# yongxuUSTC/DNN-for-speech-enhancement

Measured on AMD Instinct MI355X. Metric: training frames/sec (257x11 input, 3x2048 DNN), higher is better.
Workload: dtype f32; 1 GPU; C2: 2827->2048->2048->2048->257 ReLU+dropout(0.1/0.2), fp32, 256 frames/GPU/step (global bunch 256), lrate 1, momentum 0.5, 102400-frame chunk resident in HBM; parallelism=dp1, global_bunch=256, exchange=none, launcher=single process

## Files before the change

### dnn-for-speech-enhancement_amd/csrc/bp_device.h

```cpp
#pragma once
#include <hip/hip_runtime.h>
#include <stdint.h>

#include <type_traits>
#include <utility>

typedef float f32x16 __attribute__((ext_vector_type(16)));

template <int B, int E, class F>
__device__ __forceinline__ void static_for(F &&f)
{
    if constexpr (B < E) {
        f(std::integral_constant<int, B>{});
        static_for<B + 1, E>(std::forward<F>(f));
    }
}

__device__ __forceinline__ void philox4x32_10(uint32_t &c0, uint32_t &c1, uint32_t &c2, uint32_t &c3,
                                              uint32_t k0, uint32_t k1)
{
#pragma unroll
    for (int r = 0; r < 10; ++r) {
        const uint32_t h0 = __umulhi(0xD2511F53u, c0), l0 = 0xD2511F53u * c0;
        const uint32_t h1 = __umulhi(0xCD9E8D57u, c2), l1 = 0xCD9E8D57u * c2;
        const uint32_t n0 = h1 ^ c1 ^ k0, n2 = h0 ^ c3 ^ k1;
        c0 = n0; c1 = l1; c2 = n2; c3 = l0;
        k0 += 0x9E3779B9u; k1 += 0xBB67AE85u;
    }
}

__device__ __forceinline__ void drop_words4(uint32_t (&w)[4], int r0, int n, int frame_off, uint32_t n_true, uint32_t layer,
                                            uint32_t step, uint32_t seed_lo, uint32_t seed_hi)
{
    const uint64_t g0 = (uint64_t)(uint32_t)(r0 + frame_off);
    const uint64_t idx = (g0 >> 2) * (uint64_t)n_true + (uint32_t)n;
    uint32_t a[4] = {(uint32_t)idx, (uint32_t)(idx >> 32), layer, step};
    philox4x32_10(a[0], a[1], a[2], a[3], seed_lo, seed_hi);
    const int sh = frame_off & 3;
    if (sh == 0) { w[0] = a[0]; w[1] = a[1]; w[2] = a[2]; w[3] = a[3]; return; }
    const uint64_t idx2 = idx + (uint64_t)n_true;
    uint32_t b[4] = {(uint32_t)idx2, (uint32_t)(idx2 >> 32), layer, step};
    philox4x32_10(b[0], b[1], b[2], b[3], seed_lo, seed_hi);
    if (sh == 1) { w[0] = a[1]; w[1] = a[2]; w[2] = a[3]; w[3] = b[0]; }
    else if (sh == 2) { w[0] = a[2]; w[1] = a[3]; w[2] = b[0]; w[3] = b[1]; }
    else { w[0] = a[3]; w[1] = b[0]; w[2] = b[1]; w[3] = b[2]; }
}

__device__ __forceinline__ float act_fwd(int act, float x)
{
    return act == 0 ? (x > 0.0f ? x : 0.0f) : 1.0f / (1.0f + expf(-x));
}
__device__ __forceinline__ float act_bwd(int act, float y)
{
    return act == 0 ? (y > 0.0f ? 1.0f : 0.0f) : (1.0f - y) * y;
}

__device__ __forceinline__ float update_delta(float mom, float c1, float wc, float ndiv, float d, float g, float w)
{
    return mom * d - c1 * (g / ndiv + wc * w);
}

__device__ __forceinline__ bool last_arrival(unsigned *ticket, unsigned *lds_word, unsigned n)
{
    asm volatile("s_waitcnt vmcnt(0)" ::: "memory");
    __syncthreads();
    if (threadIdx.x == 0) *lds_word = __hip_atomic_fetch_add(ticket, 1u, __ATOMIC_RELAXED, __HIP_MEMORY_SCOPE_AGENT);
    __syncthreads();
    return (*lds_word & (n - 1)) == n - 1;
}
```

### dnn-for-speech-enhancement_amd/csrc/bp_kernels.h

```cpp
#pragma once
#include <hip/hip_runtime.h>
#include <stddef.h>
#include <stdint.h>

#include "bp_device.h"

enum { EPI_FWD_HIDDEN = 0, EPI_FWD_OUT = 1, EPI_DGRAD = 2, EPI_WGRAD_UPDATE = 3, EPI_WGRAD_STORE = 4,
       EPI_OUT_SPLIT = 6 ,
       EPI_FWD_OUT_LOGI = 7, EPI_OUT_SPLIT_LOGI = 8 };
static constexpr bool epi_out(int epi) { return epi == EPI_FWD_OUT || epi == EPI_FWD_OUT_LOGI; }
static constexpr bool epi_out_split(int epi) { return epi == EPI_OUT_SPLIT || epi == EPI_OUT_SPLIT_LOGI; }
static constexpr int OUT_SPLITS = 4;

struct GemmArgs {
    const float *A, *B;
    int lda, ldb;
    int K;
    int tiles_m, tiles_n;
#ifdef BP_TRACE
    unsigned long long *trace;
#endif
    int k_split;
    size_t slab_stride;
    float *ks_slab; unsigned *ks_ticket;
};

struct EpiArgs {
    float *C; int ldc;
    int m_limit, n_limit;
    int n_true;
    const float *bias;
    float alpha;
    int act;
    const float *aux; int ldaux;
    int lin_cols;
    float *aux2; int ldaux2;
    float scale;
    float mom, c1, wc, ndiv;
    float *bias_w, *bias_d, *bias_g;
    uint32_t drop_thresh, seed_lo, seed_hi, step, layer;
    int frame_off;
    const uint8_t *mask; int ldmask;
    int loss;
    unsigned *done;
};
static_assert(sizeof(EpiArgs) == 160 && offsetof(EpiArgs, aux2) == 56 && offsetof(EpiArgs, done) == 152, "lin_cols / loss must sit in padding");

struct EpiPre { float bias; f32x16 p0, p1; };

template <class T>
__device__ __forceinline__ T *uniform_ptr(T *p)
{
    const unsigned long long v = (unsigned long long)p;
    const unsigned lo = __builtin_amdgcn_readfirstlane((unsigned)v), hi = __builtin_amdgcn_readfirstlane((unsigned)(v >> 32));
    typedef __attribute__((address_space(1))) T *GlobalPtr;
    return (T *)(GlobalPtr)(((unsigned long long)hi << 32) | lo);
}

template <class T>
__device__ __forceinline__ T *sgpr_row_base(T *p)
{
    typedef __attribute__((address_space(1))) T *GlobalPtr;
    GlobalPtr q = (GlobalPtr)p;
    asm volatile("" : "+s"(q));
    return (T *)q;
}

template <int EPI, int R0, int RN>
__device__ __forceinline__ void epilogue_fetch(const EpiArgs &e, int mb, int nb, int lane, EpiPre &p)
{
    if constexpr (EPI == EPI_WGRAD_UPDATE) {
        const int mbc = mb < e.m_limit ? mb : 0;
        const float *cw = uniform_ptr(e.C + (size_t)mbc * e.ldc + nb);
        const float *cd = uniform_ptr(e.aux2 + (size_t)mbc * e.ldc + nb);
        const unsigned ldc = __builtin_amdgcn_readfirstlane(e.ldc);
        const unsigned lob = 4u * ((unsigned)(4 * (lane >> 5)) * (unsigned)e.ldc + (unsigned)(lane & 31));
#pragma unroll
        for (int r = R0; r < R0 + RN; ++r) {
            const unsigned ro = (unsigned)((r & 3) + 8 * (r >> 2)) * ldc;
            p.p0[r] = *reinterpret_cast<const float *>(reinterpret_cast<const char *>(sgpr_row_base(cw + ro)) + lob);
            p.p1[r] = *reinterpret_cast<const float *>(reinterpret_cast<const char *>(sgpr_row_base(cd + ro)) + lob);
        }
        return;
    }
    const int n = nb + (lane & 31);
    const int rbase = mb + 4 * (lane >> 5);
    static_assert(!epi_out_split(EPI), "fetched as EPI_FWD_OUT[_LOGI]");
    if constexpr (EPI == EPI_FWD_HIDDEN || epi_out(EPI)) p.bias = e.bias[n];
    if constexpr (epi_out(EPI) || EPI == EPI_DGRAD) {
        if (epi_out(EPI) && !e.C) return;
#pragma unroll
        for (int r = R0; r < R0 + RN; ++r) {
            const int m = rbase + (r & 3) + 8 * (r >> 2);
            const int mc = m < e.m_limit ? m : e.m_limit - 1;
            p.p0[r] = e.aux[(size_t)mc * e.ldaux + n];
        }
    }
}

template <int EPI, int R0, int RN>
__device__ __forceinline__ void epilogue_block(const EpiArgs &e, int mb, int nb, const f32x16 &acc, int lane,
                                               const EpiPre &p)
{
    static_assert(RN % 4 == 0 && R0 % 4 == 0, "register range must cover whole 4-row groups");
    if constexpr (EPI == EPI_WGRAD_UPDATE || EPI == EPI_WGRAD_STORE) {
        const int n = nb + (lane & 31);
        if (n >= e.n_limit || mb >= e.m_limit) return;
        float *cw = uniform_ptr(e.C + (size_t)mb * e.ldc + nb);
        const unsigned ldc = __builtin_amdgcn_readfirstlane(e.ldc);
        const unsigned lob = 4u * ((unsigned)(4 * (lane >> 5)) * (unsigned)e.ldc + (unsigned)(lane & 31));
#pragma unroll
        for (int r = R0; r < R0 + RN; ++r) {
            const unsigned ro = (unsigned)((r & 3) + 8 * (r >> 2)) * ldc;
            if constexpr (EPI == EPI_WGRAD_UPDATE) {
                float *cd = uniform_ptr(e.aux2 + (size_t)mb * e.ldc + nb);
                const float w = p.p0[r];
                const float d = update_delta(e.mom, e.c1, e.wc, e.ndiv, p.p1[r], acc[r], w);
                *reinterpret_cast<float *>(reinterpret_cast<char *>(sgpr_row_base(cd + ro)) + lob) = d;
                *reinterpret_cast<float *>(reinterpret_cast<char *>(sgpr_row_base(cw + ro)) + lob) = d + 1.0f * w;
            } else {
                __hip_atomic_store(reinterpret_cast<float *>(reinterpret_cast<char *>(sgpr_row_base(cw + ro)) + lob), acc[r], __ATOMIC_RELAXED, __HIP_MEMORY_SCOPE_SYSTEM);
            }
        }
        return;
    }
    const int n = nb + (lane & 31);
    const int rbase = mb + 4 * (lane >> 5);
    if (n >= e.n_limit) return;
    if constexpr (EPI == EPI_FWD_HIDDEN) {
        const float bn = p.bias;
        const bool live = n < e.n_true;
#pragma unroll
        for (int q = R0 / 4; q < (R0 + RN) / 4; ++q) {
            uint32_t w[4] = {0xFFFFFFFFu, 0xFFFFFFFFu, 0xFFFFFFFFu, 0xFFFFFFFFu};
            const int r0 = rbase + 8 * q;
            if (e.mask) {
#pragma unroll
                for (int j = 0; j < 4; ++j) w[j] = (r0 + j < e.m_limit && live && e.mask[(size_t)(r0 + j) * e.ldmask + n]) ? 0u : 0xFFFFFFFFu;
            } else if (e.drop_thresh) drop_words4(w, r0, n, e.frame_off, (uint32_t)e.n_true, e.layer, e.step, e.seed_lo, e.seed_hi);
#pragma unroll
            for (int j = 0; j < 4; ++j) {
                const int m = r0 + j;
                float y = act_fwd(e.act, e.alpha * acc[q * 4 + j] + bn);
                if (!live || w[j] < e.drop_thresh) y = 0.0f;
                if (m < e.m_limit) e.C[(size_t)m * e.ldc + n] = y;
            }
        }
    } else if constexpr (EPI == EPI_FWD_OUT) {
        const float bn = p.bias;
        const bool live = n < e.n_true;
#pragma unroll
        for (int r = R0; r < R0 + RN; ++r) {
            const int m = rbase + (r & 3) + 8 * (r >> 2);
            if (m < e.m_limit) {
                const float o = live ? e.alpha * acc[r] + bn : 0.0f;
                if (e.aux2) e.aux2[(size_t)m * e.ldaux2 + n] = o;
                if (e.C) e.C[(size_t)m * e.ldc + n] = live ? e.scale * (o - p.p0[r]) : 0.0f;
            }
        }
    } else if constexpr (EPI == EPI_FWD_OUT_LOGI) {
        const float bn = p.bias;
        const bool live = n < e.n_true, logi = live && n >= e.lin_cols, chain = logi && e.loss == 1;
#pragma unroll
        for (int r = R0; r < R0 + RN; ++r) {
            const int m = rbase + (r & 3) + 8 * (r >> 2);
            if (m < e.m_limit) {
                const float z = live ? e.alpha * acc[r] + bn : 0.0f;
                const float o = logi ? 1.0f / (1.0f + expf(-z)) : z;
                if (e.aux2) e.aux2[(size_t)m * e.ldaux2 + n] = o;
                if (e.C) {
                    float d = live ? e.scale * (o - p.p0[r]) : 0.0f;
                    if (chain) d *= o * (1.0f - o);
                    e.C[(size_t)m * e.ldc + n] = d;
                }
            }
        }
    } else if constexpr (EPI == EPI_DGRAD) {
#pragma unroll
        for (int r = R0; r < R0 + RN; ++r) {
            const int m = rbase + (r & 3) + 8 * (r >> 2);
            if (m < e.m_limit) e.C[(size_t)m * e.ldc + n] = act_bwd(e.act, p.p0[r]) * acc[r];
        }
    } else {
        static_assert(EPI == EPI_WGRAD_UPDATE || EPI == EPI_WGRAD_STORE, "epilogue without a branch");
    }
}

template <int R0>
__device__ __forceinline__ void out_split_store(const EpiArgs &e, float *slab, int mb, int nb, const f32x16 &acc, int lane)
{
    const int n = nb + (lane & 31), rbase = mb + 4 * (lane >> 5);
    if (n >= e.n_limit) return;
#pragma unroll
    for (int r = R0; r < R0 + 4; ++r) {
        const int m = rbase + (r & 3) + 8 * (r >> 2);
        if (m < e.m_limit) __hip_atomic_store(slab + (size_t)m * e.ldc + n, acc[r], __ATOMIC_RELAXED, __HIP_MEMORY_SCOPE_AGENT);
    }
}
template <int R0>
__device__ __forceinline__ void out_split_sum(const EpiArgs &e, const float *slab0, size_t stride, int mb, int nb, f32x16 &acc, int lane)
{
    const int n = nb + (lane & 31), rbase = mb + 4 * (lane >> 5);
    if (n >= e.n_limit) return;
    float p[OUT_SPLITS][4];
#pragma unroll
    for (int z = 0; z < OUT_SPLITS; ++z)
#pragma unroll
        for (int rr = 0; rr < 4; ++rr) {
            const int r = R0 + rr, m = rbase + (r & 3) + 8 * (r >> 2), mc = m < e.m_limit ? m : e.m_limit - 1;
            p[z][rr] = __hip_atomic_load(slab0 + z * stride + (size_t)mc * e.ldc + n, __ATOMIC_RELAXED, __HIP_MEMORY_SCOPE_AGENT);
        }
#pragma unroll
    for (int rr = 0; rr < 4; ++rr) {
        float s = p[0][rr];
#pragma unroll
        for (int z = 1; z < OUT_SPLITS; ++z) s += p[z][rr];
        acc[R0 + rr] = s;
    }
}

template <int KS, int KSI>
__device__ __forceinline__ void ksplit_give(const f32x16 &acc, float *red, int wq, int lane)
{
    constexpr int RN = 16 / KS;
#pragma unroll
    for (int o = 0; o < KS; ++o) {
        if (o == KSI) continue;
#pragma unroll
        for (int rr = 0; rr < RN; ++rr) red[(((wq * KS + o) * KS + KSI) * RN + rr) * 64 + lane] = acc[o * RN + rr];
    }
}
template <int KS, int KSI>
__device__ __forceinline__ void ksplit_take(f32x16 &acc, const float *red, int wq, int lane)
{
    constexpr int RN = 16 / KS;
#pragma unroll
    for (int src = 0; src < KS; ++src) {
        if (src == KSI) continue;
#pragma unroll
        for (int rr = 0; rr < RN; ++rr) acc[KSI * RN + rr] += red[(((wq * KS + KSI) * KS + src) * RN + rr) * 64 + lane];
    }
}

template <int NVA, int NVB>
struct TileRegs { float4 a[NVA]; float4 b[NVB]; };

template <int BM, int BN, int BK, int WM, int WN, bool A_KC, bool B_KC, int EPI>
struct GemmCfg {
    static constexpr int KS = 4 / (WM * WN);
    static constexpr int TM = BM / (WM * 32), TN = BN / (WN * 32);
    static constexpr int LDA_S = A_KC ? BM + 1 : BM;
    static constexpr int LDB_S = B_KC ? BN + 1 : BN;
    static constexpr int A_STAGE = (BK * LDA_S + 3) & ~3, B_STAGE = (BK * LDB_S + 3) & ~3;
    static constexpr int NVA = BM * BK / 4 / 256, NVB = BN * BK / 4 / 256;
    static constexpr int LPS = (BK / 4 < 8) ? BK / 4 : 8;
    static constexpr bool BIASG = (EPI == EPI_WGRAD_UPDATE || EPI == EPI_WGRAD_STORE);
    static_assert(WM * WN * KS == 4 && TM >= 1 && TN >= 1, "wave layout");
    static_assert(BK % (2 * KS) == 0 && BK % 4 == 0, "BK");
    static_assert(NVA >= 1 && NVB >= 1, "tile too small for 256 threads");
    using Regs = TileRegs<NVA, NVB>;

    struct Offs { int a[NVA]; int b[NVB]; };
    static __device__ __forceinline__ void make_offs(Offs &o, const GemmArgs &g, int tid)
    {
#pragma unroll
        for (int i = 0; i < NVA; ++i) {
            const int f = tid + i * 256;
            if constexpr (A_KC) {
                const int l8 = f % LPS, seg = f / LPS, row = seg % BM, k4 = (seg / BM) * LPS + l8;
                o.a[i] = row * g.lda + k4 * 4;
            } else {
                const int c4 = f % (BM / 4), k = f / (BM / 4);
                o.a[i] = k * g.lda + c4 * 4;
            }
        }
#pragma unroll
        for (int i = 0; i < NVB; ++i) {
            const int f = tid + i * 256;
            if constexpr (B_KC) {
                const int l8 = f % LPS, seg = f / LPS, row = seg % BN, k4 = (seg / BN) * LPS + l8;
                o.b[i] = row * g.ldb + k4 * 4;
            } else {
                const int c4 = f % (BN / 4), k = f / (BN / 4);
                o.b[i] = k * g.ldb + c4 * 4;
            }
        }
    }
    static __device__ __forceinline__ const float *base_a(const GemmArgs &g, int m0, int k0)
    {
        return A_KC ? g.A + (size_t)m0 * g.lda + k0 : g.A + (size_t)k0 * g.lda + m0;
    }
    static __device__ __forceinline__ const float *base_b(const GemmArgs &g, int n0, int k0)
    {
        return B_KC ? g.B + (size_t)n0 * g.ldb + k0 : g.B + (size_t)k0 * g.ldb + n0;
    }
    static __device__ __forceinline__ void load_a(Regs &r, int i, const float *pa, const Offs &o)
    {
        r.a[i] = *reinterpret_cast<const float4 *>(pa + o.a[i]);
    }
    static __device__ __forceinline__ void load_b(Regs &r, int i, const float *pb, const Offs &o)
    {
        r.b[i] = *reinterpret_cast<const float4 *>(pb + o.b[i]);
    }
    static __device__ __forceinline__ void load(Regs &r, const float *pa, const float *pb, const Offs &o)
    {
#pragma unroll
        for (int i = 0; i < NVA; ++i) load_a(r, i, pa, o);
#pragma unroll
        for (int i = 0; i < NVB; ++i) load_b(r, i, pb, o);
    }

    static __device__ __forceinline__ void store_a(const Regs &r, int i, float *As, int tid)
    {
        const int f = tid + i * 256;
        const float4 v = r.a[i];
        if constexpr (A_KC) {
            const int l8 = f % LPS, seg = f / LPS, row = seg % BM, k4 = (seg / BM) * LPS + l8;
            As[(k4 * 4 + 0) * LDA_S + row] = v.x; As[(k4 * 4 + 1) * LDA_S + row] = v.y;
            As[(k4 * 4 + 2) * LDA_S + row] = v.z; As[(k4 * 4 + 3) * LDA_S + row] = v.w;
        } else {
            const int c4 = f % (BM / 4), k = f / (BM / 4);
            *reinterpret_cast<float4 *>(As + k * LDA_S + c4 * 4) = v;
        }
    }
    static __device__ __forceinline__ void store_b(const Regs &r, int i, float *Bs, int tid, float4 &bsum)
    {
        const int f = tid + i * 256;
        const float4 v = r.b[i];
        if constexpr (B_KC) {
            const int l8 = f % LPS, seg = f / LPS, row = seg % BN, k4 = (seg / BN) * LPS + l8;
            Bs[(k4 * 4 + 0) * LDB_S + row] = v.x; Bs[(k4 * 4 + 1) * LDB_S + row] = v.y;
            Bs[(k4 * 4 + 2) * LDB_S + row] = v.z; Bs[(k4 * 4 + 3) * LDB_S + row] = v.w;
        } else {
            const int c4 = f % (BN / 4), k = f / (BN / 4);
            *reinterpret_cast<float4 *>(Bs + k * LDB_S + c4 * 4) = v;
            if constexpr (BIASG) {
                bsum.x += v.x; bsum.y += v.y; bsum.z += v.z; bsum.w += v.w;
            }
        }
    }
    static __device__ __forceinline__ void store(const Regs &r, float *As, float *Bs, int tid, float4 &bsum)
    {
#pragma unroll
        for (int i = 0; i < NVA; ++i) store_a(r, i, As, tid);
#pragma unroll
        for (int i = 0; i < NVB; ++i) store_b(r, i, Bs, tid, bsum);
    }

    static constexpr int NCH = (TM * TN == 1) ? 2 : 1;
    template <bool DO_STORE, bool DO_LOAD>
    static __device__ __forceinline__ void step(const float *As, const float *Bs, f32x16 (&acc)[NCH][TM][TN], int ks,
                                                int a_off, int b_off, int kh, const Regs &rs, float *AsN, float *BsN,
                                                Regs &rl, const float *pa, const float *pb, const Offs &o, int tid,
                                                float4 &bsum)
    {
        constexpr int NK = BK / KS / 2, NP = NVA + NVB, RD = NK < 4 ? NK : 4;
        const float *ap = As + (ks * (BK / KS) + kh) * LDA_S + a_off;
        const float *bp = Bs + (ks * (BK / KS) + kh) * LDB_S + b_off;
        float av[NK][TM], bv[NK][TN];
        __builtin_amdgcn_sched_barrier(0);
#pragma unroll
        for (int s = 0; s < RD; ++s) {
#pragma unroll
            for (int i = 0; i < TM; ++i) av[s][i] = ap[2 * s * LDA_S + i * 32];
#pragma unroll
            for (int j = 0; j < TN; ++j) bv[s][j] = bp[2 * s * LDB_S + j * 32];
        }
        __builtin_amdgcn_sched_barrier(0);
        int pl = 0, ps = 0;
#pragma unroll
        for (int s = 0; s < NK; ++s) {
#pragma unroll
            for (int i = 0; i < TM; ++i)
#pragma unroll
                for (int j = 0; j < TN; ++j)
                    acc[s % NCH][i][j] = __builtin_amdgcn_mfma_f32_32x32x2f32(av[s][i], bv[s][j], acc[s % NCH][i][j], 0, 0, 0);
            if (s + RD < NK) {
#pragma unroll
                for (int i = 0; i < TM; ++i) av[s + RD][i] = ap[2 * (s + RD) * LDA_S + i * 32];
#pragma unroll
                for (int j = 0; j < TN; ++j) bv[s + RD][j] = bp[2 * (s + RD) * LDB_S + j * 32];
            }
            if constexpr (DO_LOAD) {
#pragma unroll
                for (int q = 0; q < NP; ++q) {
                    if (q == pl && (q * NK) / NP == s) {
                        if (q < NVA) load_a(rl, q, pa, o); else load_b(rl, q - NVA, pb, o);
                        ++pl;
                    }
                }
            }
            if constexpr (DO_STORE) {
#pragma unroll
                for (int q = 0; q < NP; ++q) {
                    if (q == ps && (q * NK) / NP == s) {
                        if (q < NVA) store_a(rs, q, AsN, tid); else store_b(rs, q - NVA, BsN, tid, bsum);
                        ++ps;
                    }
                }
            }
            __builtin_amdgcn_sched_barrier(0);
        }
    }
};

template <int BM, int BN, int BK, int WM, int WN, bool A_KC, bool B_KC, int EPI>
struct GemmKernel {
    using Cfg = GemmCfg<BM, BN, BK, WM, WN, A_KC, B_KC, EPI>;
    static constexpr int KS = Cfg::KS, TM = Cfg::TM, TN = Cfg::TN;
    static constexpr int A_STAGE = Cfg::A_STAGE, B_STAGE = Cfg::B_STAGE, STAGE = A_STAGE + B_STAGE;
    static constexpr bool BIASG = Cfg::BIASG;
    static constexpr int RED = (KS > 1) ? KS * WM * WN * 16 * 64 : 0;
    static constexpr int BIASRED = BIASG ? 256 / (BN / 4) * BN : 0;
    static constexpr int SMEM0 = (2 * STAGE > RED) ? 2 * STAGE : RED;
    static constexpr int SMEM = SMEM0 > BIASRED ? SMEM0 : BIASRED;
    static constexpr int MIN_WG = (SMEM * 4 > 80 * 1024) ? 1 : 2;

static __device__ __forceinline__ void run(const GemmArgs &g_in, const EpiArgs &e_in, int first_block, int stride,
                                           int block_y, float *smem)
{
    using Regs = typename Cfg::Regs;
    const int tid = threadIdx.x, lane = tid & 63, wave = __builtin_amdgcn_readfirstlane(tid >> 6);
    const int ks = wave / (WM * WN), wq = wave % (WM * WN), wm = wq / WN, wn = wq % WN;
    GemmArgs g = g_in;
    EpiArgs e = e_in;
    constexpr int EPI_E = EPI == EPI_OUT_SPLIT ? EPI_FWD_OUT : EPI == EPI_OUT_SPLIT_LOGI ? EPI_FWD_OUT_LOGI : EPI;
    if constexpr (epi_out_split(EPI)) {
        const size_t kz = (size_t)block_y * g.k_split;
        g.A += A_KC ? kz : kz * g.lda;
        g.B += B_KC ? kz : kz * g.ldb;
    }

#ifdef BP_TRACE
#define TRACE(i) do { if (tid == 0 && g.trace) { g.trace[(size_t)first_block * 8 + (i)] = wall_clock64();                 \
        if ((i) == 0) g.trace[(size_t)first_block * 8 + 6] = clock64();                 \
        if ((i) == 3) g.trace[(size_t)first_block * 8 + 7] = clock64();              \
    } } while (0)
#else
#define TRACE(i) ((void)0)
#endif
    TRACE(0);
    for (int b = first_block; b < g.tiles_m * g.tiles_n; b += stride) {
    int tile_m, tile_n;
    {
        if ((g.tiles_n & 7) == 0) {
            const int xcd = b & 7, j = b >> 3, per = g.tiles_n >> 3;
            if constexpr (BIASG) {
                tile_n = xcd * per + j % per;
                tile_m = j / per;
            } else {
                tile_n = xcd * per + j / g.tiles_m;
                tile_m = j % g.tiles_m;
            }
        } else {
            tile_m = b % g.tiles_m;
            tile_n = b / g.tiles_m;
        }
    }
    const int m0 = tile_m * BM, n0 = tile_n * BN;

    float4 bsum = make_float4(0.f, 0.f, 0.f, 0.f);
    const bool do_bias = BIASG && tile_m == 0;

    constexpr int NCH = Cfg::NCH;
    f32x16 accs[NCH][TM][TN];
#pragma unroll
    for (int c = 0; c < NCH; ++c)
#pragma unroll
        for (int i = 0; i < TM; ++i)
#pragma unroll
            for (int j = 0; j < TN; ++j)
#pragma unroll
                for (int r = 0; r < 16; ++r) accs[c][i][j][r] = 0.0f;

    const int nt = (g.K + BK - 1) / BK;
    const int a_off = wm * TM * 32 + (lane & 31), b_off = wn * TN * 32 + (lane & 31);
    const int kh = lane >> 5;

    EpiPre pre[TM][TN];
    const int mb0 = m0 + wm * TM * 32, nb0 = n0 + wn * TN * 32;
    if constexpr (KS == 1) {
#pragma unroll
        for (int i = 0; i < TM; ++i)
#pragma unroll
            for (int j = 0; j < TN; ++j) epilogue_fetch<EPI_E, 0, 16>(e, mb0 + i * 32, nb0 + j * 32, lane, pre[i][j]);
    } else {
        static_assert(KS == 1 || (TM == 1 && TN == 1), "in-workgroup k-split needs one block per wave");
        if (ks == 0) epilogue_fetch<EPI_E, 0, 16 / KS>(e, mb0, nb0, lane, pre[0][0]);
        if (ks == 1) epilogue_fetch<EPI_E, 16 / KS, 16 / KS>(e, mb0, nb0, lane, pre[0][0]);
        if constexpr (KS == 4) {
            if (ks == 2) epilogue_fetch<EPI_E, 8, 4>(e, mb0, nb0, lane, pre[0][0]);
            if (ks == 3) epilogue_fetch<EPI_E, 12, 4>(e, mb0, nb0, lane, pre[0][0]);
        }
    }

    const int last_k0 = (nt - 1) * BK;
    typename Cfg::Offs offs;
    Cfg::make_offs(offs, g, tid);
#define K0_OF(t) (((t) * BK) < last_k0 ? ((t) * BK) : last_k0)
#define PA(t) Cfg::base_a(g, m0, K0_OF(t))
#define PB(t) Cfg::base_b(g, n0, K0_OF(t))
#define AS(buf) (smem + (buf) * STAGE)
#define BS(buf) (smem + (buf) * STAGE + A_STAGE)
#define STEP(ST, LD, buf, RS, RL, TL)                                                                      \
    Cfg::template step<ST, LD>(AS(buf), BS(buf), accs, ks, a_off, b_off, kh, RS, AS((buf) ^ 1), BS((buf) ^ 1),    \
                               RL, PA(TL), PB(TL), offs, tid, bsum)
    Regs r0, r1;
    Cfg::load(r0, PA(0), PB(0), offs);
    Cfg::store(r0, AS(0), BS(0), tid, bsum);
    Cfg::load(r1, PA(1), PB(1), offs);
    __syncthreads();
    TRACE(1);
    int t = 0, buf = 0;
    for (; t + 3 <= nt; t += 2) {
        STEP(true, true, 0, r1, r0, t + 2);
        __syncthreads();
        STEP(true, true, 1, r0, r1, t + 3);
        __syncthreads();
    }
    if (nt - t == 2) {
        STEP(true, false, 0, r1, r0, 0);
        __syncthreads();
        buf = 1;
    }
    STEP(false, false, buf, r0, r0, 0);
    __syncthreads();
    TRACE(2);
#undef K0_OF
#undef PA
#undef PB
#undef AS
#undef BS
#undef STEP
    f32x16 (&acc)[TM][TN] = accs[0];
    if constexpr (NCH == 2) {
#pragma unroll
        for (int i = 0; i < TM; ++i)
#pragma unroll
            for (int j = 0; j < TN; ++j)
#pragma unroll
                for (int r = 0; r < 16; ++r) acc[i][j][r] += accs[1][i][j][r];
    }

    if constexpr (KS > 1) {
        if (ks == 0) ksplit_give<KS, 0>(acc[0][0], smem, wq, lane);
        if (ks == 1) ksplit_give<KS, 1>(acc[0][0], smem, wq, lane);
        if constexpr (KS == 4) {
            if (ks == 2) ksplit_give<KS, 2>(acc[0][0], smem, wq, lane);
            if (ks == 3) ksplit_give<KS, 3>(acc[0][0], smem, wq, lane);
        }
        __syncthreads();
        if (ks == 0) ksplit_take<KS, 0>(acc[0][0], smem, wq, lane);
        if (ks == 1) ksplit_take<KS, 1>(acc[0][0], smem, wq, lane);
        if constexpr (KS == 4) {
            if (ks == 2) ksplit_take<KS, 2>(acc[0][0], smem, wq, lane);
            if (ks == 3) ksplit_take<KS, 3>(acc[0][0], smem, wq, lane);
        }
        if constexpr (BIASG) __syncthreads();
    }

    if constexpr (BIASG && !B_KC) {
        if (do_bias) {
            constexpr int CG = BN / 4, RG = 256 / CG;
            float *red = smem;
            const int c4 = tid % CG, rg = tid / CG;
            *reinterpret_cast<float4 *>(red + rg * BN + c4 * 4) = bsum;
            __syncthreads();
            if (tid < BN && (n0 + tid) < e.n_limit) {
                float s = 0.f;
#pragma unroll
                for (int r = 0; r < RG; ++r) s += red[r * BN + tid];
                const int n = n0 + tid;
                if constexpr (EPI == EPI_WGRAD_UPDATE) {
                    const float d = update_delta(e.mom, e.c1, 0.0f, e.ndiv, e.bias_d[n], s, e.bias_w[n]);
                    e.bias_d[n] = d;
                    e.bias_w[n] = d + 1.0f * e.bias_w[n];
                } else {
                    e.bias_g[n] = s;
                }
            }
        }
    }

    bool finish = true;
    if constexpr (epi_out_split(EPI)) {
        static_assert(KS == 4 && OUT_SPLITS == 4, "one 32x32 block per workgroup, four registers of it per wave");
        float *mine = g.ks_slab + (size_t)block_y * g.slab_stride;
        if (ks == 0) out_split_store<0>(e, mine, mb0, nb0, acc[0][0], lane);
        if (ks == 1) out_split_store<4>(e, mine, mb0, nb0, acc[0][0], lane);
        if (ks == 2) out_split_store<8>(e, mine, mb0, nb0, acc[0][0], lane);
        if (ks == 3) out_split_store<12>(e, mine, mb0, nb0, acc[0][0], lane);
        finish = last_arrival(g.ks_ticket + b, reinterpret_cast<unsigned *>(smem), OUT_SPLITS);
        if (finish) {
            if (ks == 0) out_split_sum<0>(e, g.ks_slab, g.slab_stride, mb0, nb0, acc[0][0], lane);
            if (ks == 1) out_split_sum<4>(e, g.ks_slab, g.slab_stride, mb0, nb0, acc[0][0], lane);
            if (ks == 2) out_split_sum<8>(e, g.ks_slab, g.slab_stride, mb0, nb0, acc[0][0], lane);
            if (ks == 3) out_split_sum<12>(e, g.ks_slab, g.slab_stride, mb0, nb0, acc[0][0], lane);
        }
    }

    if constexpr (KS == 1) {
#pragma unroll
        for (int i = 0; i < TM; ++i)
#pragma unroll
            for (int j = 0; j < TN; ++j)
                epilogue_block<EPI_E, 0, 16>(e, mb0 + i * 32, nb0 + j * 32, acc[i][j], lane, pre[i][j]);
    } else if (finish) {
        if (ks == 0) epilogue_block<EPI_E, 0, 16 / KS>(e, mb0, nb0, acc[0][0], lane, pre[0][0]);
        if (ks == 1) epilogue_block<EPI_E, 16 / KS, 16 / KS>(e, mb0, nb0, acc[0][0], lane, pre[0][0]);
        if constexpr (KS == 4) {
            if (ks == 2) epilogue_block<EPI_E, 8, 4>(e, mb0, nb0, acc[0][0], lane, pre[0][0]);
            if (ks == 3) epilogue_block<EPI_E, 12, 4>(e, mb0, nb0, acc[0][0], lane, pre[0][0]);
        }
    }
    if (b + stride < g.tiles_m * g.tiles_n) __syncthreads();
    }
    TRACE(3);
#undef TRACE
}
};

template <int BM, int BN, int BK, int WM, int WN, bool A_KC, bool B_KC, int EPI, int TAG = 0>
__global__ __launch_bounds__(256, (GemmKernel<BM, BN, BK, WM, WN, A_KC, B_KC, EPI>::MIN_WG)) void bp_gemm(const GemmArgs g, const EpiArgs e)
{
    using K = GemmKernel<BM, BN, BK, WM, WN, A_KC, B_KC, EPI>;
    __shared__ __attribute__((aligned(16))) float smem[K::SMEM];
    K::run(g, e, blockIdx.x, gridDim.x, blockIdx.y, smem);
}

struct MultiArgs {
    GemmArgs g[4];
    EpiArgs e[4];
    int first_tile[5];
    int n;
};
template <class K>
__global__ __launch_bounds__(256, K::MIN_WG) void bp_gemm_multi(const MultiArgs a)
{
    __shared__ __attribute__((aligned(16))) float smem[K::SMEM];
    const int b = blockIdx.x;
    int p = 0;
    while (p + 1 < a.n && b >= a.first_tile[p + 1]) ++p;
    K::run(a.g[p], a.e[p], b - a.first_tile[p], a.first_tile[p + 1] - a.first_tile[p], 0, smem);
}

struct StageArgs {
    float *x; int ld, width;
    const float *fea; int fea_dim, win;
    const float *nat; const int *win_start, *nat_row;
    int rows; uint32_t thresh; int frame_off; uint32_t seed_lo, seed_hi, step;
    float *t; int ldt, twidth; const float *targ_frames; const int *targ_frame;
    int yb_in;
    int nbx;
};
__device__ __forceinline__ void stage_rows_block(const StageArgs &a, int bx, int by, int tx)
{
    const int r0 = bx * 4, c = (by * 256 + tx) * 4;
    if (c >= a.ld) return;
    float4 v[4];
#pragma unroll
    for (int j = 0; j < 4; ++j)
        v[j] = *reinterpret_cast<const float4 *>(a.fea + (size_t)(r0 + j < a.rows ? r0 + j : a.rows - 1) * a.fea_dim + c);
    if (a.thresh) {
        uint32_t drop = 0;
#pragma unroll 1
        for (int k = 0; k < 4; ++k) {
            if (c + k >= a.width) break;
            uint32_t w[4];
            drop_words4(w, r0, c + k, a.frame_off, (uint32_t)a.width, 0u, a.step, a.seed_lo, a.seed_hi);
            const uint32_t m = (w[0] < a.thresh ? 1u : 0u) | (w[1] < a.thresh ? 2u : 0u) | (w[2] < a.thresh ? 4u : 0u) | (w[3] < a.thresh ? 8u : 0u);
            drop |= m << (4 * k);
        }
#pragma unroll
        for (int j = 0; j < 4; ++j) {
            if (drop & (1u << (0 + j))) v[j].x = 0.0f;
            if (drop & (1u << (4 + j))) v[j].y = 0.0f;
            if (drop & (1u << (8 + j))) v[j].z = 0.0f;
            if (drop & (1u << (12 + j))) v[j].w = 0.0f;
        }
    }
#pragma unroll
    for (int j = 0; j < 4; ++j) if (r0 + j < a.rows) *reinterpret_cast<float4 *>(a.x + (size_t)(r0 + j) * a.ld + c) = v[j];
}
__device__ __forceinline__ void stage_block(const StageArgs &a, int bx, int by, int tx)
{
    if (!a.win_start) { stage_rows_block(a, bx, by, tx); return; }
    const int r0 = bx * 4;
    float v[4] = {0.0f, 0.0f, 0.0f, 0.0f};
    int rr[4];
#pragma unroll
    for (int j = 0; j < 4; ++j) rr[j] = r0 + j < a.rows ? r0 + j : a.rows - 1;
    if (by >= a.yb_in) {
        const int c = (by - a.yb_in) * 256 + tx;
        if (c >= a.ldt) return;
        if (c < a.twidth) {
            int tf[4];
#pragma unroll
            for (int j = 0; j < 4; ++j) tf[j] = a.targ_frame[rr[j]];
#pragma unroll
            for (int j = 0; j < 4; ++j) v[j] = a.targ_frames[(size_t)tf[j] * a.twidth + c];
        }
#pragma unroll
        for (int j = 0; j < 4; ++j) if (r0 + j < a.rows) a.t[(size_t)(r0 + j) * a.ldt + c] = v[j];
        return;
    }
    const int c = by * 256 + tx;
    if (c >= a.ld) return;
    if (c < a.win) {
        int ws[4];
#pragma unroll
        for (int j = 0; j < 4; ++j) ws[j] = a.win_start[rr[j]];
#pragma unroll
        for (int j = 0; j < 4; ++j) v[j] = a.fea[(size_t)ws[j] * a.fea_dim + c];
    } else if (c < a.width) {
        int nr[4];
#pragma unroll
        for (int j = 0; j < 4; ++j) nr[j] = a.nat_row[rr[j]];
#pragma unroll
        for (int j = 0; j < 4; ++j) v[j] = a.nat[(size_t)nr[j] * a.fea_dim + (c - a.win)];
    }
    uint32_t w[4] = {~0u, ~0u, ~0u, ~0u};
    if (a.thresh && c < a.width) drop_words4(w, r0, c, a.frame_off, (uint32_t)a.width, 0u, a.step, a.seed_lo, a.seed_hi);
#pragma unroll
    for (int j = 0; j < 4; ++j) if (r0 + j < a.rows) a.x[(size_t)(r0 + j) * a.ld + c] = w[j] < a.thresh ? 0.0f : v[j];
}
__global__ __launch_bounds__(256) void bp_stage_bunch(const StageArgs a)
{
    stage_block(a, blockIdx.x % a.nbx, blockIdx.x / a.nbx, threadIdx.x);
}

__global__ void bp_apply_mask(const float *in, float *out, int ld, int width, const uint8_t *mask, int n_frames)
{
    const int u = blockIdx.x * blockDim.x + threadIdx.x, f = blockIdx.y;
    if (u >= ld || f >= n_frames) return;
    float v = in[(size_t)f * ld + u];
    if (u < width && mask[(size_t)f * width + u]) v = 0.0f;
    out[(size_t)f * ld + u] = v;
}

__global__ void bp_fill_normal(float *buf, int ld, int width, int rows, uint32_t seed_lo, uint32_t seed_hi,
                               uint32_t stream)
{
    const size_t i = (size_t)blockIdx.x * blockDim.x + threadIdx.x;
    const size_t per_row = (size_t)(ld / 4);
    if (i >= per_row * (size_t)rows) return;
    const size_t r = i / per_row; const int c = (int)(i % per_row) * 4;
    uint32_t w0 = (uint32_t)i, w1 = (uint32_t)(i >> 32), w2 = stream, w3 = 0x5EEDu;
    philox4x32_10(w0, w1, w2, w3, seed_lo, seed_hi);
    const float u0 = (w0 + 1.0f) * 2.3283064365386963e-10f, u1 = w1 * 2.3283064365386963e-10f;
    const float u2 = (w2 + 1.0f) * 2.3283064365386963e-10f, u3 = w3 * 2.3283064365386963e-10f;
    const float r0 = sqrtf(-2.0f * logf(fminf(u0, 1.0f))), r1 = sqrtf(-2.0f * logf(fminf(u2, 1.0f)));
    float v[4] = { r0 * cosf(6.283185307179586f * u1), r0 * sinf(6.283185307179586f * u1),
                   r1 * cosf(6.283185307179586f * u3), r1 * sinf(6.283185307179586f * u3) };
    float4 o;
    o.x = (c + 0 < width) ? v[0] : 0.f; o.y = (c + 1 < width) ? v[1] : 0.f;
    o.z = (c + 2 < width) ? v[2] : 0.f; o.w = (c + 3 < width) ? v[3] : 0.f;
    *reinterpret_cast<float4 *>(buf + r * ld + c) = o;
}

template <class K>
__global__ __launch_bounds__(256, K::MIN_WG) void bp_out_split_stage(const GemmArgs g, const EpiArgs e, int n_gemm, const StageArgs st)
{
    __shared__ __attribute__((aligned(16))) float smem[K::SMEM];
    const int b = blockIdx.x;
    if (b < n_gemm) { const int tiles = g.tiles_m * g.tiles_n; K::run(g, e, b % tiles, tiles, b / tiles, smem); }
    else { const int i = b - n_gemm; stage_block(st, i % st.nbx, i / st.nbx, threadIdx.x); }
}
```

Baseline: 1.189 million frames/s.

## Precompute dropout mask bits during prologue load latency, use SGPR-based block stores

Moves the Philox dropout RNG draws for the forward hidden epilogue into the GEMM prologue, between the issue of the first two tile loads and the LDS store, so the RNG arithmetic overlaps global-memory latency. The draws are packed into a per-lane bitmask held in EpiPre. The hidden and dgrad epilogue stores now use SGPR row bases with a lane byte offset whenever the whole 32-row block is in range. The weight-update stores also become relaxed atomic stores. The cost is extra live registers across the main loop and a reordered prologue, which may lower occupancy.

```diff
diff --git a/dnn-for-speech-enhancement_amd/csrc/bp_device.h b/dnn-for-speech-enhancement_amd/csrc/bp_device.h
--- a/dnn-for-speech-enhancement_amd/csrc/bp_device.h
+++ b/dnn-for-speech-enhancement_amd/csrc/bp_device.h
@@ -46,6 +46,21 @@
     else { w[0] = a[3]; w[1] = b[0]; w[2] = b[1]; w[3] = b[2]; }
 }
 
+template <int NQ>
+__device__ __forceinline__ uint32_t drop_bits(int r0, int n, int frame_off, uint32_t n_true, uint32_t layer, uint32_t step,
+                                              uint32_t seed_lo, uint32_t seed_hi, uint32_t thresh)
+{
+    uint32_t bits = 0;
+#pragma unroll 1
+    for (int q = 0; q < NQ; ++q) {
+        uint32_t w[4];
+        drop_words4(w, r0 + 8 * q, n, frame_off, n_true, layer, step, seed_lo, seed_hi);
+        const uint32_t m = (w[0] < thresh ? 1u : 0u) | (w[1] < thresh ? 2u : 0u) | (w[2] < thresh ? 4u : 0u) | (w[3] < thresh ? 8u : 0u);
+        bits |= m << (4 * q);
+    }
+    return bits;
+}
+
 __device__ __forceinline__ float act_fwd(int act, float x)
 {
     return act == 0 ? (x > 0.0f ? x : 0.0f) : 1.0f / (1.0f + expf(-x));
diff --git a/dnn-for-speech-enhancement_amd/csrc/bp_kernels.h b/dnn-for-speech-enhancement_amd/csrc/bp_kernels.h
--- a/dnn-for-speech-enhancement_amd/csrc/bp_kernels.h
+++ b/dnn-for-speech-enhancement_amd/csrc/bp_kernels.h
@@ -46,7 +46,7 @@
 };
 static_assert(sizeof(EpiArgs) == 160 && offsetof(EpiArgs, aux2) == 56 && offsetof(EpiArgs, done) == 152, "lin_cols / loss must sit in padding");
 
-struct EpiPre { float bias; f32x16 p0, p1; };
+struct EpiPre { float bias; uint32_t drop; f32x16 p0, p1; };
 
 template <class T>
 __device__ __forceinline__ T *uniform_ptr(T *p)
@@ -64,6 +64,31 @@
     GlobalPtr q = (GlobalPtr)p;
     asm volatile("" : "+s"(q));
     return (T *)q;
+}
+
+template <class T>
+__device__ __forceinline__ T &block_elem(T *block, unsigned row, unsigned lob)
+{
+    return *(T *)((const char *)sgpr_row_base(block + row) + lob);
+}
+
+template <int R0, int RN>
+__device__ __forceinline__ void block_store(const EpiArgs &e, int mb, int nb, int lane, const float (&v)[RN])
+{
+    if (mb + 32 <= e.m_limit) {
+        float *c = uniform_ptr(e.C + (size_t)mb * e.ldc + nb);
+        const unsigned ldc = __builtin_amdgcn_readfirstlane(e.ldc);
+        const unsigned lob = 4u * ((unsigned)(4 * (lane >> 5)) * (unsigned)e.ldc + (unsigned)(lane & 31));
+#pragma unroll
+        for (int r = R0; r < R0 + RN; ++r) block_elem(c, (unsigned)((r & 3) + 8 * (r >> 2)) * ldc, lob) = v[r - R0];
+    } else {
+        const int n = nb + (lane & 31), rbase = mb + 4 * (lane >> 5);
+#pragma unroll
+        for (int r = R0; r < R0 + RN; ++r) {
+            const int m = rbase + (r & 3) + 8 * (r >> 2);
+            if (m < e.m_limit) e.C[(size_t)m * e.ldc + n] = v[r - R0];
+        }
+    }
 }
 
 template <int EPI, int R0, int RN>
@@ -96,6 +121,15 @@
             p.p0[r] = e.aux[(size_t)mc * e.ldaux + n];
         }
     }
+}
+
+template <int RN>
+__device__ __forceinline__ void epilogue_draw(const EpiArgs &e, int mb, int nb, int lane, int r_first, EpiPre &p)
+{
+    p.drop = 0;
+    if (e.drop_thresh && !e.mask)
+        p.drop = drop_bits<RN / 4>(mb + 4 * (lane >> 5) + 2 * r_first, nb + (lane & 31), e.frame_off, (uint32_t)e.n_true, e.layer, e.step,
+                                   e.seed_lo, e.seed_hi, e.drop_thresh);
 }
 
 template <int EPI, int R0, int RN>
@@ -116,8 +150,8 @@
                 float *cd = uniform_ptr(e.aux2 + (size_t)mb * e.ldc + nb);
                 const float w = p.p0[r];
                 const float d = update_delta(e.mom, e.c1, e.wc, e.ndiv, p.p1[r], acc[r], w);
-                *reinterpret_cast<float *>(reinterpret_cast<char *>(sgpr_row_base(cd + ro)) + lob) = d;
-                *reinterpret_cast<float *>(reinterpret_cast<char *>(sgpr_row_base(cw + ro)) + lob) = d + 1.0f * w;
+                __hip_atomic_store(reinterpret_cast<float *>(reinterpret_cast<char *>(sgpr_row_base(cd + ro)) + lob), d, __ATOMIC_RELAXED, __HIP_MEMORY_SCOPE_AGENT);
+                __hip_atomic_store(reinterpret_cast<float *>(reinterpret_cast<char *>(sgpr_row_base(cw + ro)) + lob), d + 1.0f * w, __ATOMIC_RELAXED, __HIP_MEMORY_SCOPE_AGENT);
             } else {
                 __hip_atomic_store(reinterpret_cast<float *>(reinterpret_cast<char *>(sgpr_row_base(cw + ro)) + lob), acc[r], __ATOMIC_RELAXED, __HIP_MEMORY_SCOPE_SYSTEM);
             }
@@ -130,22 +164,22 @@
     if constexpr (EPI == EPI_FWD_HIDDEN) {
         const float bn = p.bias;
         const bool live = n < e.n_true;
+        float y[RN];
 #pragma unroll
         for (int q = R0 / 4; q < (R0 + RN) / 4; ++q) {
-            uint32_t w[4] = {0xFFFFFFFFu, 0xFFFFFFFFu, 0xFFFFFFFFu, 0xFFFFFFFFu};
+            uint32_t drop = p.drop >> (4 * q - R0);
             const int r0 = rbase + 8 * q;
             if (e.mask) {
 #pragma unroll
-                for (int j = 0; j < 4; ++j) w[j] = (r0 + j < e.m_limit && live && e.mask[(size_t)(r0 + j) * e.ldmask + n]) ? 0u : 0xFFFFFFFFu;
-            } else if (e.drop_thresh) drop_words4(w, r0, n, e.frame_off, (uint32_t)e.n_true, e.layer, e.step, e.seed_lo, e.seed_hi);
+                for (int j = 0; j < 4; ++j) drop |= (r0 + j < e.m_limit && live && e.mask[(size_t)(r0 + j) * e.ldmask + n] && e.drop_thresh) ? 1u << j : 0u;
+            }
 #pragma unroll
             for (int j = 0; j < 4; ++j) {
-                const int m = r0 + j;
-                float y = act_fwd(e.act, e.alpha * acc[q * 4 + j] + bn);
-                if (!live || w[j] < e.drop_thresh) y = 0.0f;
-                if (m < e.m_limit) e.C[(size_t)m * e.ldc + n] = y;
-            }
-        }
+                y[q * 4 + j - R0] = act_fwd(e.act, e.alpha * acc[q * 4 + j] + bn);
+                if (!live || (drop >> j & 1u)) y[q * 4 + j - R0] = 0.0f;
+            }
+        }
+        block_store<R0, RN>(e, mb, nb, lane, y);
     } else if constexpr (EPI == EPI_FWD_OUT) {
         const float bn = p.bias;
         const bool live = n < e.n_true;
@@ -176,11 +210,10 @@
             }
         }
     } else if constexpr (EPI == EPI_DGRAD) {
-#pragma unroll
-        for (int r = R0; r < R0 + RN; ++r) {
-            const int m = rbase + (r & 3) + 8 * (r >> 2);
-            if (m < e.m_limit) e.C[(size_t)m * e.ldc + n] = act_bwd(e.act, p.p0[r]) * acc[r];
-        }
+        float d[RN];
+#pragma unroll
+        for (int r = R0; r < R0 + RN; ++r) d[r - R0] = act_bwd(e.act, p.p0[r]) * acc[r];
+        block_store<R0, RN>(e, mb, nb, lane, d);
     } else {
         static_assert(EPI == EPI_WGRAD_UPDATE || EPI == EPI_WGRAD_STORE, "epilogue without a branch");
     }
@@ -507,8 +540,23 @@
                                RL, PA(TL), PB(TL), offs, tid, bsum)
     Regs r0, r1;
     Cfg::load(r0, PA(0), PB(0), offs);
-    Cfg::store(r0, AS(0), BS(0), tid, bsum);
-    Cfg::load(r1, PA(1), PB(1), offs);
+    if constexpr (EPI_E == EPI_FWD_HIDDEN) {
+        Cfg::load(r1, PA(1), PB(1), offs);
+        __builtin_amdgcn_sched_barrier(0);
+        if constexpr (KS == 1) {
+#pragma unroll
+            for (int i = 0; i < TM; ++i)
+#pragma unroll
+                for (int j = 0; j < TN; ++j) epilogue_draw<16>(e, mb0 + i * 32, nb0 + j * 32, lane, 0, pre[i][j]);
+        } else {
+            epilogue_draw<16 / KS>(e, mb0, nb0, lane, ks * (16 / KS), pre[0][0]);
+        }
+        __builtin_amdgcn_sched_barrier(0);
+        Cfg::store(r0, AS(0), BS(0), tid, bsum);
+    } else {
+        Cfg::store(r0, AS(0), BS(0), tid, bsum);
+        Cfg::load(r1, PA(1), PB(1), offs);
+    }
     __syncthreads();
     TRACE(1);
     int t = 0, buf = 0;
```

Result: no change. 1.196 million frames/s, median of 6 (+0.6%).
